# MegviiRobot/CamLaserCalibraTool

Hardware: AMD Instinct MI355X
Metric: residual+Jacobian evals/s (LM solve, 1e6-obs synthetic point-to-plane problem per GPU) (higher is better)
Workload: dtype f64

## Files before the change

camlasercalibratool_amd/csrc/clc_coop.hpp:

```cpp
#pragma once
#include "clc_lmuni.hpp"
#include "clc_resident.hpp"

namespace clc {

constexpr int COOP_WGS = 256, COOP_GROUPS = 8, COOP_PER_GROUP = COOP_WGS / COOP_GROUPS, COOP_ROW_WORDS = 64;
constexpr int COOP_SMALL_WGS = 32;
#ifndef CLC_COOP_A_STRIDE
#define CLC_COOP_A_STRIDE 64
#endif
#ifndef CLC_COOP_B_STRIDE
#define CLC_COOP_B_STRIDE 64
#endif
constexpr int COOP_A_STRIDE = CLC_COOP_A_STRIDE, COOP_B_STRIDE = CLC_COOP_B_STRIDE;
constexpr int COOP_NW = 4, COOP_NL = 64 * COOP_NW;
constexpr int COOP_THREADS = COOP_NL + 64;
constexpr int COOP_STATUS_ABORT = -1;
constexpr int COOP_PR = 16, COOP_PL = 24;
constexpr int COOP_PR_Z = 10, COOP_PL_Z = 16;
constexpr unsigned long long COOP_CENSUS_TICKS = 20000ull;
constexpr unsigned long long COOP_TIMEOUT_TICKS = 100000ull;
constexpr int COOP_DONE_OK = 1, COOP_DONE_ABORT = 2;
#ifndef CLC_COOP_POLL_SLEEP
#define CLC_COOP_POLL_SLEEP 1
#endif
#ifndef CLC_COOP_D1
#define CLC_COOP_D1 900
#endif
#ifndef CLC_COOP_D2
#define CLC_COOP_D2 2200
#endif

#ifndef CLC_COOP_GRP
#define CLC_COOP_GRP 8
#endif
#ifndef CLC_COOP_REPLICAS
#define CLC_COOP_REPLICAS 1
#endif
constexpr int COOP_REPLICAS = CLC_COOP_REPLICAS;
constexpr unsigned long long COOP_ABORT_CHECK_TICKS = 2000ull;
struct CoopBoard {
  unsigned long long a[2][COOP_WGS][COOP_A_STRIDE];
  unsigned long long b[2][COOP_REPLICAS][COOP_GROUPS][COOP_B_STRIDE];
  unsigned long long ctl[8];
};

typedef unsigned int v4u __attribute__((ext_vector_type(4)));
constexpr int COOP_SC1 = 16;
__device__ __forceinline__ __amdgpu_buffer_rsrc_t coop_rsrc(CoopBoard* board) {
  return __builtin_amdgcn_make_buffer_rsrc(board, 0, (int)sizeof(CoopBoard), 0x00020000);
}
__device__ __forceinline__ void coop_put(__amdgpu_buffer_rsrc_t rs, const unsigned int row_byte, const int e, const double v, const unsigned int tag) {
  v4u w;
  w[0] = tag; w[1] = (unsigned int)__double2hiint(v); w[2] = tag; w[3] = (unsigned int)__double2loint(v);
  __builtin_amdgcn_raw_buffer_store_b128(w, rs, row_byte + 16u * (unsigned int)e, 0, COOP_SC1);
}
__device__ __forceinline__ v4u coop_get(__amdgpu_buffer_rsrc_t rs, const unsigned int byte) {
  return __builtin_amdgcn_raw_buffer_load_b128(rs, byte, 0, COOP_SC1);
}
__device__ __forceinline__ bool coop_valid(const v4u w, const unsigned int tag) { return w[0] == tag && w[2] == tag; }
__device__ __forceinline__ double coop_value(const v4u w) { return __hiloint2double((int)w[1], (int)w[3]); }
__device__ __forceinline__ unsigned int coop_row_a(const int par, const int wg) {
  return (unsigned int)(offsetof(CoopBoard, a) + ((size_t)(par * COOP_WGS + wg) * COOP_A_STRIDE) * 8);
}
__device__ __forceinline__ unsigned int coop_row_b(const int par, const int copy, const int grp) {
  return (unsigned int)(offsetof(CoopBoard, b) + ((size_t)((par * COOP_REPLICAS + copy) * COOP_GROUPS + grp) * COOP_B_STRIDE) * 8);
}
__device__ __forceinline__ void coop_wait_until(const long long t) {
  while (clock64() < t) __builtin_amdgcn_s_sleep(2);
}

#ifdef CLC_STAMPS
constexpr int COOP_STAMP_PASSES = 16, COOP_STAMP_PER_PASS = 12, COOP_STAMP_SLOTS = COOP_STAMP_PER_PASS * COOP_STAMP_PASSES + 2;
static __device__ long long clc_coop_stamp_buf[4][2][COOP_STAMP_SLOTS];
#define COOP_STAMP(slot)                                                                                                     \
  do {                                                                                                                       \
    if (lane == 0 && (wave == 0 || wave >= COOP_NW - 1) && (wg == 0 || wg == 7 || wg == 8 || wg == 255) && (slot) < COOP_STAMP_SLOTS)  \
      clc_coop_stamp_buf[wg == 0 ? 0 : wg == 7 ? 1 : wg == 8 ? 2 : 3][wave == COOP_NW - 1 ? 1 : 0][slot] = clock64();          \
  } while (0)
#else
#define COOP_STAMP(slot) do {} while (0)
#endif

__device__ __forceinline__ void wave_reduce_to_rows(double (&acc)[NACC], double (&u)[7]) {
  double r[14];
#pragma unroll
  for (int i = 0; i < 14; ++i) {
    double x = acc[i], y = acc[i + 14];
    swap_halves(x, y);
    r[i] = x + y;
  }
#pragma unroll
  for (int i = 0; i < 7; ++i) {
    double x = r[i], y = r[i + 7];
    swap_rows(x, y);
    u[i] = x + y;
  }
}

template <bool WITH_LOSS, bool NT, bool WITH_Z = false, bool ONE_HOP = false>
__global__ __launch_bounds__(COOP_THREADS) void coop_solve_kernel(
    const double* __restrict__ xyl, const double* __restrict__ zl, const unsigned int* __restrict__ res_row, const ResLane* __restrict__ lane_desc,
    const double* __restrict__ groups, const int uni_ppl, const clc_options opt, const Pose7 pose0, clc_iteration* __restrict__ trace,
    const int trace_cap, CoopBoard* __restrict__ board, const unsigned int tag0, double* __restrict__ pose_out,
    clc_summary* __restrict__ summary_out, double* __restrict__ results, int32_t* __restrict__ host_done, const int n_wgs) {
  constexpr int NW = COOP_NW, NL = COOP_NL, PR = WITH_Z ? COOP_PR_Z : COOP_PR, PL = WITH_Z ? COOP_PL_Z : COOP_PL, NP = PR + PL;
  constexpr int CH = WITH_Z ? 4 : 6, NCH = (PL + CH - 1) / CH;
  static_assert(NW == 4, "the row tail maps the four 16-lane rows of a wave onto the four point waves");
  using Moments = typename std::conditional<WITH_Z, RowMoments3, RowMoments>::type;
  __shared__ v2d sh_pts[PL * NL];
  __shared__ double sh_ptz[WITH_Z ? PL * NL : 1];
  __shared__ double sh_state[LM_STATE_WORDS];
  __shared__ __attribute__((aligned(16))) double sh_tot[64];
  __shared__ double sh_red[NW * 7 * 64];
  __shared__ __attribute__((aligned(16))) double sh_pub[LM_PUB_WORDS];
  const int wg = blockIdx.x, tid = threadIdx.x, lane = tid & 63, wave = tid >> 6;
  const int cap = opt.max_num_iterations + 2;
#ifdef CLC_STAMPS
  int stamp_pass = 0;
  COOP_STAMP(COOP_STAMP_PER_PASS * COOP_STAMP_PASSES);
#endif

  if (wave == NW) {
    constexpr bool one_hop = ONE_HOP;
    constexpr int groups = ONE_HOP ? 1 : COOP_GROUPS;
    const int grp = ONE_HOP ? 0 : wg % COOP_GROUPS;
    const bool leader = ONE_HOP || wg < COOP_GROUPS;
    clc_iteration* const tr = wg == 0 ? trace : nullptr;
    const int tr_cap = wg == 0 ? trace_cap : 0;
    LmState& st = *reinterpret_cast<LmState*>(sh_state);
    const __amdgpu_buffer_rsrc_t rs = coop_rsrc(board);
    LmU S;
    {
      double x0[7];
#pragma unroll
      for (int i = 0; i < 7; ++i) x0[i] = pose0.v[i];
      lmu_init(S, st, opt, x0, lane);
      lmu_publish(sh_pub, x0, CLC_RUNNING, lane);
    }
    __syncthreads();
    bool aborted = false;

    const long long d1 = board->ctl[1] ? (long long)board->ctl[1] : (ONE_HOP ? 1900 : CLC_COOP_D1), d2 = board->ctl[2] ? (long long)board->ctl[2] : CLC_COOP_D2;
    for (int k = 0;; ++k) {
      __syncthreads();
      const unsigned int tag = tag0 + (unsigned int)k;
      const int par = k & 1;
      const int h = lane >> 5, e = (lane & 31) < NACC ? (lane & 31) : NACC - 1;
      const bool mine = lane < NACC;
      const unsigned long long limit = k == 0 ? COOP_CENSUS_TICKS : COOP_TIMEOUT_TICKS;
      bool fine = true;
      const long long t_a = clock64();
      if (ONE_HOP) {
        if (k > 0) lmu_pre(S, st, opt, sh_tot, tr, tr_cap, lane);
        COOP_STAMP(COOP_STAMP_PER_PASS * stamp_pass + 11);
      }
      if (leader) {
        coop_wait_until(t_a + d1);
        v4u w[16];
        const unsigned int base = coop_row_a(par, grp + groups * 16 * h) + 16u * (unsigned int)e;
        constexpr unsigned int row_step = (unsigned int)(groups * COOP_A_STRIDE * 8);
        const unsigned long long t0 = wall_clock64();
        for (;;) {
          bool ok = true;
          unsigned int bo = base;
          asm volatile("" : "+v"(bo));
#pragma unroll
          for (int i = 0; i < 16; ++i) w[i] = coop_get(rs, bo + (unsigned int)i * row_step);
#pragma unroll
          for (int i = 0; i < 16; ++i) ok = ok && coop_valid(w[i], tag);
          if (__all(ok)) break;
          const unsigned long long waited = wall_clock64() - t0;
          if (waited > COOP_ABORT_CHECK_TICKS) {
            unsigned int co = (unsigned int)offsetof(CoopBoard, ctl);
            asm volatile("" : "+v"(co));
            if (waited > limit || coop_get(rs, co)[0] == tag0) { fine = false; break; }
          }
          __builtin_amdgcn_s_sleep(CLC_COOP_POLL_SLEEP);
        }
        COOP_STAMP(COOP_STAMP_PER_PASS * stamp_pass + 3);
        double s = coop_value(w[0]);
#pragma unroll
        for (int i = 1; i < 16; ++i) s += coop_value(w[i]);
        double s_lo = s, s_hi = s;
        swap_halves(s_lo, s_hi);
        if (one_hop) {
          if (mine) sh_tot[32 * (1 - S.hx) + lane] = s_lo + s_hi;
        } else if (mine && fine) {
          int so = lane;
          asm volatile("" : "+v"(so));
#pragma unroll
          for (int r = 0; r < COOP_REPLICAS; ++r) coop_put(rs, coop_row_b(par, (r + grp) % COOP_REPLICAS, grp), so, s_lo + s_hi, tag);
        }
        COOP_STAMP(COOP_STAMP_PER_PASS * stamp_pass + 4);
      }
      if (!ONE_HOP) {
        if (k > 0 && !leader) lmu_pre(S, st, opt, sh_tot, tr, tr_cap, lane);
        if (!leader) COOP_STAMP(COOP_STAMP_PER_PASS * stamp_pass + 11);
      }
      if (fine && !one_hop) {
        coop_wait_until(t_a + d2);
        const unsigned int base = coop_row_b(par, wg % COOP_REPLICAS, 4 * h) + 16u * (unsigned int)e;
        const unsigned long long t0 = wall_clock64();
        bool pre_due = k > 0 && leader;
        v4u w[4];
        for (;;) {
          bool ok = true;
          unsigned int bo = base;
          asm volatile("" : "+v"(bo));
#pragma unroll
          for (int i = 0; i < 4; ++i) w[i] = coop_get(rs, bo + (unsigned int)(i * COOP_B_STRIDE * 8));
          if (pre_due) {
            asm volatile("" ::: "memory");
            __builtin_amdgcn_sched_barrier(0);
            lmu_pre(S, st, opt, sh_tot, tr, tr_cap, lane);
            __builtin_amdgcn_sched_barrier(0);
            COOP_STAMP(COOP_STAMP_PER_PASS * stamp_pass + 11);
            pre_due = false;
          }
#pragma unroll
          for (int i = 0; i < 4; ++i) ok = ok && coop_valid(w[i], tag);
          if (__all(ok)) break;
          const unsigned long long waited = wall_clock64() - t0;
          if (waited > COOP_ABORT_CHECK_TICKS) {
            unsigned int co = (unsigned int)offsetof(CoopBoard, ctl);
            asm volatile("" : "+v"(co));
            if (waited > limit || coop_get(rs, co)[0] == tag0) { fine = false; break; }
          }
          __builtin_amdgcn_s_sleep(CLC_COOP_POLL_SLEEP);
        }
        COOP_STAMP(COOP_STAMP_PER_PASS * stamp_pass + 5);
        double s = coop_value(w[0]);
#pragma unroll
        for (int i = 1; i < 4; ++i) s += coop_value(w[i]);
        double s_lo = s, s_hi = s;
        swap_halves(s_lo, s_hi);
        if (mine) sh_tot[32 * (1 - S.hx) + lane] = s_lo + s_hi;
      }
      __builtin_amdgcn_fence(__ATOMIC_RELEASE, "wavefront");
      __builtin_amdgcn_wave_barrier();
      __builtin_amdgcn_fence(__ATOMIC_ACQUIRE, "wavefront");
      COOP_STAMP(COOP_STAMP_PER_PASS * stamp_pass + 6);
      if (fine) {
        lmu_post(k == 0, S, opt, sh_tot, sh_pub, tr, tr_cap, lane);
        if (S.status == CLC_RUNNING && k >= cap) {
          S.status = CLC_FAILURE;
          lmu_publish_status(sh_pub, CLC_FAILURE, lane);
        }
      } else {
        if (lane == 0) __hip_atomic_store(reinterpret_cast<unsigned int*>(&board->ctl[0]), tag0, __ATOMIC_RELAXED, __HIP_MEMORY_SCOPE_AGENT);
        lmu_publish_status(sh_pub, COOP_STATUS_ABORT, lane);
        aborted = true;
      }
      COOP_STAMP(COOP_STAMP_PER_PASS * stamp_pass + 7);
      __syncthreads();
      if (aborted || S.status != CLC_RUNNING) break;
#ifdef CLC_STAMPS
      ++stamp_pass;
#endif
    }
    if (wg == 0) {
      if (!aborted) {
        lmu_finish(S, st, opt, sh_tot, tr, tr_cap, lane);
        if (lane == 0) batched_write_outcome(st, 0, pose_out, summary_out, results);
      }
      if (lane == 0) __hip_atomic_store(host_done, aborted ? COOP_DONE_ABORT : COOP_DONE_OK, __ATOMIC_RELEASE, __HIP_MEMORY_SCOPE_SYSTEM);
    }
    return;
  }

  __builtin_amdgcn_s_setprio(2);
  const __amdgpu_buffer_rsrc_t rs_p = coop_rsrc(board);
  unsigned int row0;
  int ppl;
  if (uni_ppl >= 0) {
    row0 = (unsigned int)wg * (unsigned int)uni_ppl;
    ppl = uni_ppl;
  } else {
    row0 = res_row[wg];
    ppl = __builtin_amdgcn_readfirstlane((int)(res_row[wg + 1] - row0));
  }
  const ResLane dl = lane_desc[(size_t)wg * NL + tid];
  const v2d* __restrict__ src = reinterpret_cast<const v2d*>(xyl) + (size_t)row0 * NL + tid;
  const int j_last = ppl > 0 ? ppl - 1 : 0;
  const double* __restrict__ srcz = WITH_Z ? zl + (size_t)row0 * NL + tid : nullptr;
  v2d lds_v[PL];
  double lds_z[WITH_Z ? PL : 1];
  const bool use_lds = (ppl + CLC_COOP_GRP - 1) / CLC_COOP_GRP * CLC_COOP_GRP > PR;
  if (use_lds) {
#pragma unroll
    for (int i = 0; i < PL; ++i) {
      const int j = PR + i;
      lds_v[i] = res_load<NT>(src + (size_t)(j < j_last ? j : j_last) * NL);
      if (WITH_Z) lds_z[i] = srcz[(size_t)(j < j_last ? j : j_last) * NL];
    }
  }
  v2d reg[PR];
  double regz[WITH_Z ? PR : 1];
#pragma unroll
  for (int j = 0; j < PR; ++j) {
    reg[j] = res_load<NT>(src + (size_t)(j < j_last ? j : j_last) * NL);
    if (WITH_Z) regz[j] = srcz[(size_t)(j < j_last ? j : j_last) * NL];
  }
  if (use_lds) {
#pragma unroll
    for (int i = 0; i < PL; ++i) {
      v2d v = lds_v[i];
      double vz = WITH_Z ? lds_z[i] : 0.0;
      if (PR + i >= ppl) { v[0] = 0.0; v[1] = 0.0; vz = 0.0; }
      sh_pts[i * NL + tid] = v;
      if (WITH_Z) sh_ptz[i * NL + tid] = vz;
    }
  }
  const double* __restrict__ gp = groups + (size_t)dl.gid * GROUP_DOUBLES;
  const int cnt = dl.cnt;
  double pl_nx = 0.0, pl_ny = 0.0, pl_nz = 0.0, pl_d = 0.0, pl_s2 = 0.0;
  if (cnt > 0) {
    const v2d a = *reinterpret_cast<const v2d*>(gp);
    const v2d b = *reinterpret_cast<const v2d*>(gp + 2);
    const double s = gp[4];
    pl_nx = a[0]; pl_ny = a[1]; pl_nz = b[0]; pl_d = b[1]; pl_s2 = s * s;
  }
  const double inv_lf2 = make_uniform(1.0 / (opt.loss_scale_factor * opt.loss_scale_factor));
  constexpr int GRP = CLC_COOP_GRP;
  const int ppl_up = (ppl + GRP - 1) / GRP * GRP;
  const int ppl_eff = ppl_up < NP ? ppl_up : NP;
#ifndef CLC_COOP_PAD_ANALYTIC
#define CLC_COOP_PAD_ANALYTIC 0
#endif
  constexpr bool PAD_ANALYTIC = CLC_COOP_PAD_ANALYTIC != 0;
  static_assert(!(PAD_ANALYTIC && WITH_Z), "the analytic padding correction is written for (x, y) slots only");
  const int cnt_m = cnt > 0 ? cnt : ppl_eff;
  int cmin = cnt_m;
#pragma unroll
  for (int off = 32; off >= 1; off >>= 1) {
    const int o2 = __shfl_xor(cmin, off, 64);
    cmin = o2 < cmin ? o2 : cmin;
  }
  cmin = __builtin_amdgcn_readfirstlane(cmin);
  __syncthreads();
  COOP_STAMP(COOP_STAMP_PER_PASS * COOP_STAMP_PASSES + 1);
#pragma unroll
  for (int j = 0; j < PR; ++j)
    if (j >= ppl) { reg[j][0] = 0.0; reg[j][1] = 0.0; if (WITH_Z) regz[j] = 0.0; }

  for (int k = 0;; ++k) {
    COOP_STAMP(COOP_STAMP_PER_PASS * stamp_pass);
    int t = tid;
    asm volatile("" : "+v"(t));
    RowPlane q;
    {
      const lds_cv2d* pb = lds_opaque(sh_pub);
      const v2d p0 = pb[0], p1 = pb[1], p2 = pb[2], p3 = pb[3], p4 = pb[4], p5 = pb[5], p6 = pb[6];
      int status = __double2loint(p6[0]);
      asm volatile("" : "+v"(status) : "v"(p0), "v"(p1), "v"(p2), "v"(p3), "v"(p4), "v"(p5));
      if (status != CLC_RUNNING) break;
      q.nx = pl_nx; q.ny = pl_ny; q.nz = pl_nz; q.s2 = pl_s2;
      q.mx = fma(p3[0], pl_nz, fma(p1[1], pl_ny, p0[0] * pl_nx));
      q.my = fma(p3[1], pl_nz, fma(p2[0], pl_ny, p0[1] * pl_nx));
      q.mz = fma(p4[0], pl_nz, fma(p2[1], pl_ny, p1[0] * pl_nx));
      q.c0 = fma(p5[1], pl_nz, fma(p5[0], pl_ny, fma(p4[1], pl_nx, pl_d)));
    }
    v2d buf[2][CH];
    double bufz[2][WITH_Z ? CH : 1];
    if (use_lds) {
#pragma unroll
      for (int u = 0; u < CH; ++u)
        if (u < PL) {
          buf[0][u] = sh_pts[u * NL + t];
          if (WITH_Z) bufz[0][u] = sh_ptz[u * NL + t];
        }
    }
#ifdef CLC_STAMPS
    asm volatile("" :: "v"(q.mx), "v"(q.c0));
    COOP_STAMP(COOP_STAMP_PER_PASS * stamp_pass + 8);
#endif
    Moments M;
    lane_moments_reset<WITH_LOSS>(M);
#pragma unroll
    for (int j0 = 0; j0 < NP; j0 += GRP) {
      if (j0 < ppl) {
        if (PAD_ANALYTIC || j0 + GRP <= cmin) {
#pragma unroll
          for (int j = j0; j < j0 + GRP && j < NP; ++j) {
            if (j >= PR && (j - PR) % CH == 0 && (j - PR) / CH + 1 < NCH) {
              const int c1 = (j - PR) / CH + 1;
#pragma unroll
              for (int u = 0; u < CH; ++u)
                if (c1 * CH + u < PL) {
                  buf[c1 & 1][u] = sh_pts[(c1 * CH + u) * NL + t];
                  if (WITH_Z) bufz[c1 & 1][u] = sh_ptz[(c1 * CH + u) * NL + t];
                }
            }
            const v2d v = j < PR ? reg[j < PR ? j : 0] : buf[((j - PR) / CH) & 1][(j - PR) % CH];
            const double vz = !WITH_Z ? 0.0 : (j < PR ? regz[j < PR ? j : 0] : bufz[((j - PR) / CH) & 1][(j - PR) % CH]);
            lane_point<WITH_LOSS>(q, inv_lf2, v[0], v[1], vz, M, j == j0 + GRP - 1);
          }
        } else {
#pragma unroll
          for (int j = j0; j < j0 + GRP && j < NP; ++j) {
            if (j >= PR && (j - PR) % CH == 0 && (j - PR) / CH + 1 < NCH) {
              const int c1 = (j - PR) / CH + 1;
#pragma unroll
              for (int u = 0; u < CH; ++u)
                if (c1 * CH + u < PL) {
                  buf[c1 & 1][u] = sh_pts[(c1 * CH + u) * NL + t];
                  if (WITH_Z) bufz[c1 & 1][u] = sh_ptz[(c1 * CH + u) * NL + t];
                }
            }
            const v2d v = j < PR ? reg[j < PR ? j : 0] : buf[((j - PR) / CH) & 1][(j - PR) % CH];
            const double vz = !WITH_Z ? 0.0 : (j < PR ? regz[j < PR ? j : 0] : bufz[((j - PR) / CH) & 1][(j - PR) % CH]);
            lane_point_masked<WITH_LOSS>(q, j < cnt_m, inv_lf2, v[0], v[1], vz, M, j == j0 + GRP - 1);
          }
        }
      }
    }
    double lp = 0.0;
    if (PAD_ANALYTIC) {
      const int npad = ppl_eff - cnt;
      const double np = (double)npad;
      const double c0 = q.c0;
      if (WITH_LOSS) {
        const double sum_p = fma(c0 * c0, inv_lf2, 1.0);
        const double w_p = rcp_ge1(sum_p);
        const double cs = npad > 0 ? np * w_p : 0.0;
        M.S0 -= cs;
        M.T0 = fma(-cs, c0, M.T0);
        int e;
        const double m = frexp_pos(sum_p, e);
        lp = npad > 0 ? np * log_mant_exp(m, e) : 0.0;
      } else {
        const double cs = npad > 0 ? np : 0.0;
        M.S0 -= cs;
        M.T0 = fma(-cs, c0, M.T0);
        M.prod = fma(-cs * c0, c0, M.prod);
      }
    } else {
      lane_pad_correction<WITH_LOSS>(M, (double)(ppl_eff - cnt_m));
    }
#ifdef CLC_STAMPS
    asm volatile("" :: "v"(M.S0), "v"(M.Tx), "v"(M.prod));
    COOP_STAMP(COOP_STAMP_PER_PASS * stamp_pass + 9);
#endif
    double acc[NACC];
#pragma unroll
    for (int i = 0; i < NACC; ++i) acc[i] = 0.0;
    lane_flush<WITH_LOSS>(q, M, acc);
    if (PAD_ANALYTIC && WITH_LOSS) acc[27] = fma(-q.s2, lp, acc[27]);
#ifdef CLC_STAMPS
    asm volatile("" :: "v"(acc[0]), "v"(acc[20]), "v"(acc[27]));
    COOP_STAMP(COOP_STAMP_PER_PASS * stamp_pass + 10);
#endif
    {
      double u[7];
      wave_reduce_to_rows(acc, u);
#pragma unroll
      for (int i = 0; i < 7; ++i) sh_red[(wave * 7 + i) * 64 + lane] = u[i];
    }
    COOP_STAMP(COOP_STAMP_PER_PASS * stamp_pass + 1);
    __syncthreads();
    {
      const unsigned int tag = tag0 + (unsigned int)k;
      const int s0 = ((lane >> 4) * 7) * 64 + 16 * wave + (lane & 15);
      double v[8];
#pragma unroll
      for (int i = 0; i < 7; ++i) v[i] = sh_red[s0 + i * 64];
      v[7] = 0.0;
      double r[4], s[2];
#pragma unroll
      for (int i = 0; i < 4; ++i) {
        double x = v[i], y = v[i + 4];
        swap_halves(x, y);
        r[i] = x + y;
      }
#pragma unroll
      for (int i = 0; i < 2; ++i) {
        double x = r[i], y = r[i + 2];
        swap_rows(x, y);
        s[i] = x + y;
      }
#pragma unroll
      for (int i = 0; i < 2; ++i) {
        double w = s[i];
        w += dpp_read<0xB1>(w);
        w += dpp_read<0x4E>(w);
        w += dpp_read<0x141>(w);
        w += dpp_read<0x140>(w);
        s[i] = w;
      }
      if ((lane & 15) == 0) {
        const int rho = lane >> 4;
        const unsigned int row = coop_row_a(k & 1, wg);
#pragma unroll
        for (int i = 0; i < 2; ++i) {
          const int e = i + 2 * (rho & 1) + 4 * (rho >> 1);
          if (e < 7) coop_put(rs_p, row, 7 * wave + e, s[i], tag);
        }
      }
    }
    COOP_STAMP(COOP_STAMP_PER_PASS * stamp_pass + 2);
    __syncthreads();
#ifdef CLC_STAMPS
    ++stamp_pass;
#endif
  }
}

}
```

Baseline: 154.4 billion.

## Move group-leader gather into a dedicated extra wave per workgroup

Adds a sixth wave to each workgroup that, on the first COOP_GROUPS workgroups, polls the stage-A board rows, sums the group partials and publishes them to the stage-B board. The control wave no longer does the leader gather itself, so every workgroup runs lmu_pre and the stage-B poll the same way and the leader's pre-step work no longer serialises with its gather. The D1/D2 spin delays are retuned to fit the new timing. In exchange each workgroup launches 64 more threads, which adds register and occupancy pressure and extra __syncthreads coordination between the waves.

Result: faster. 159.7 billion, median of 6 (+3.4%).

```diff
diff --git a/camlasercalibratool_amd/csrc/clc_coop.hpp b/camlasercalibratool_amd/csrc/clc_coop.hpp
--- a/camlasercalibratool_amd/csrc/clc_coop.hpp
+++ b/camlasercalibratool_amd/csrc/clc_coop.hpp
@@ -14,7 +14,7 @@
 #endif
 constexpr int COOP_A_STRIDE = CLC_COOP_A_STRIDE, COOP_B_STRIDE = CLC_COOP_B_STRIDE;
 constexpr int COOP_NW = 4, COOP_NL = 64 * COOP_NW;
-constexpr int COOP_THREADS = COOP_NL + 64;
+constexpr int COOP_THREADS = COOP_NL + 128;
 constexpr int COOP_STATUS_ABORT = -1;
 constexpr int COOP_PR = 16, COOP_PL = 24;
 constexpr int COOP_PR_Z = 10, COOP_PL_Z = 16;
@@ -25,10 +25,10 @@
 #define CLC_COOP_POLL_SLEEP 1
 #endif
 #ifndef CLC_COOP_D1
-#define CLC_COOP_D1 900
+#define CLC_COOP_D1 1200
 #endif
 #ifndef CLC_COOP_D2
-#define CLC_COOP_D2 2200
+#define CLC_COOP_D2 1400
 #endif
 
 #ifndef CLC_COOP_GRP
@@ -96,6 +96,44 @@
     swap_rows(x, y);
     u[i] = x + y;
   }
+}
+
+template <int NR>
+__device__ __forceinline__ bool coop_poll(const __amdgpu_buffer_rsrc_t rs, const unsigned int base, const unsigned int step, const unsigned int tag,
+                                          const unsigned int tag0, const unsigned long long limit, v4u (&w)[NR]) {
+  const unsigned long long t0 = wall_clock64();
+  for (;;) {
+    bool ok = true;
+    unsigned int bo = base;
+    asm volatile("" : "+v"(bo));
+#pragma unroll
+    for (int i = 0; i < NR; ++i) w[i] = coop_get(rs, bo + (unsigned int)i * step);
+#pragma unroll
+    for (int i = 0; i < NR; ++i) ok = ok && coop_valid(w[i], tag);
+    if (__all(ok)) return true;
+    const unsigned long long waited = wall_clock64() - t0;
+    if (waited > COOP_ABORT_CHECK_TICKS) {
+      unsigned int co = (unsigned int)offsetof(CoopBoard, ctl);
+      asm volatile("" : "+v"(co));
+      if (waited > limit || coop_get(rs, co)[0] == tag0) return false;
+    }
+    __builtin_amdgcn_s_sleep(CLC_COOP_POLL_SLEEP);
+  }
+}
+
+template <int GROUPS>
+__device__ __forceinline__ bool coop_gather_group(const __amdgpu_buffer_rsrc_t rs, const int par, const int grp, const int lane, const unsigned int tag,
+                                                  const unsigned int tag0, const unsigned long long limit, double& row) {
+  const int h = lane >> 5, e = (lane & 31) < NACC ? (lane & 31) : NACC - 1;
+  v4u w[16];
+  const bool fine = coop_poll<16>(rs, coop_row_a(par, grp + GROUPS * 16 * h) + 16u * (unsigned int)e, (unsigned int)(GROUPS * COOP_A_STRIDE * 8), tag, tag0, limit, w);
+  double s = coop_value(w[0]);
+#pragma unroll
+  for (int i = 1; i < 16; ++i) s += coop_value(w[i]);
+  double s_lo = s, s_hi = s;
+  swap_halves(s_lo, s_hi);
+  row = s_lo + s_hi;
+  return fine;
 }
 
 template <bool WITH_LOSS, bool NT, bool WITH_Z = false, bool ONE_HOP = false>
@@ -121,11 +159,39 @@
   COOP_STAMP(COOP_STAMP_PER_PASS * COOP_STAMP_PASSES);
 #endif
 
+  if (wave == NW + 1) {
+    if (ONE_HOP || wg >= COOP_GROUPS) return;
+    const __amdgpu_buffer_rsrc_t rs = coop_rsrc(board);
+    const long long d1 = board->ctl[1] ? (long long)board->ctl[1] : CLC_COOP_D1;
+    const int grp = wg;
+    __syncthreads();
+    for (int k = 0;; ++k) {
+      __syncthreads();
+      const long long t_a = clock64();
+      const unsigned int tag = tag0 + (unsigned int)k;
+      const int par = k & 1;
+      coop_wait_until(t_a + d1);
+      double row;
+      const bool fine = coop_gather_group<COOP_GROUPS>(rs, par, grp, lane, tag, tag0, k == 0 ? COOP_CENSUS_TICKS : COOP_TIMEOUT_TICKS, row);
+      COOP_STAMP(COOP_STAMP_PER_PASS * stamp_pass + 3);
+      if (fine) {
+        if (lane < NACC) {
+#pragma unroll
+          for (int r = 0; r < COOP_REPLICAS; ++r) coop_put(rs, coop_row_b(par, (r + grp) % COOP_REPLICAS, grp), lane, row, tag);
+        }
+      } else if (lane == 0) {
+        __hip_atomic_store(reinterpret_cast<unsigned int*>(&board->ctl[0]), tag0, __ATOMIC_RELAXED, __HIP_MEMORY_SCOPE_AGENT);
+      }
+      COOP_STAMP(COOP_STAMP_PER_PASS * stamp_pass + 4);
+      __syncthreads();
+      if (reinterpret_cast<const volatile int*>(sh_pub + 12)[0] != CLC_RUNNING) return;
+#ifdef CLC_STAMPS
+      ++stamp_pass;
+#endif
+    }
+  }
+
   if (wave == NW) {
-    constexpr bool one_hop = ONE_HOP;
-    constexpr int groups = ONE_HOP ? 1 : COOP_GROUPS;
-    const int grp = ONE_HOP ? 0 : wg % COOP_GROUPS;
-    const bool leader = ONE_HOP || wg < COOP_GROUPS;
     clc_iteration* const tr = wg == 0 ? trace : nullptr;
     const int tr_cap = wg == 0 ? trace_cap : 0;
     LmState& st = *reinterpret_cast<LmState*>(sh_state);
@@ -141,94 +207,28 @@
     __syncthreads();
     bool aborted = false;
 
-    const long long d1 = board->ctl[1] ? (long long)board->ctl[1] : (ONE_HOP ? 1900 : CLC_COOP_D1), d2 = board->ctl[2] ? (long long)board->ctl[2] : CLC_COOP_D2;
+    const long long d = ONE_HOP ? (board->ctl[1] ? (long long)board->ctl[1] : 1900) : (board->ctl[2] ? (long long)board->ctl[2] : CLC_COOP_D2);
     for (int k = 0;; ++k) {
       __syncthreads();
       const unsigned int tag = tag0 + (unsigned int)k;
       const int par = k & 1;
-      const int h = lane >> 5, e = (lane & 31) < NACC ? (lane & 31) : NACC - 1;
       const bool mine = lane < NACC;
       const unsigned long long limit = k == 0 ? COOP_CENSUS_TICKS : COOP_TIMEOUT_TICKS;
-      bool fine = true;
+      bool fine;
       const long long t_a = clock64();
+      if (k > 0) lmu_pre(S, st, opt, sh_tot, tr, tr_cap, lane);
+      COOP_STAMP(COOP_STAMP_PER_PASS * stamp_pass + 11);
+      coop_wait_until(t_a + d);
       if (ONE_HOP) {
-        if (k > 0) lmu_pre(S, st, opt, sh_tot, tr, tr_cap, lane);
-        COOP_STAMP(COOP_STAMP_PER_PASS * stamp_pass + 11);
-      }
-      if (leader) {
-        coop_wait_until(t_a + d1);
-        v4u w[16];
-        const unsigned int base = coop_row_a(par, grp + groups * 16 * h) + 16u * (unsigned int)e;
-        constexpr unsigned int row_step = (unsigned int)(groups * COOP_A_STRIDE * 8);
-        const unsigned long long t0 = wall_clock64();
-        for (;;) {
-          bool ok = true;
-          unsigned int bo = base;
-          asm volatile("" : "+v"(bo));
-#pragma unroll
-          for (int i = 0; i < 16; ++i) w[i] = coop_get(rs, bo + (unsigned int)i * row_step);
-#pragma unroll
-          for (int i = 0; i < 16; ++i) ok = ok && coop_valid(w[i], tag);
-          if (__all(ok)) break;
-          const unsigned long long waited = wall_clock64() - t0;
-          if (waited > COOP_ABORT_CHECK_TICKS) {
-            unsigned int co = (unsigned int)offsetof(CoopBoard, ctl);
-            asm volatile("" : "+v"(co));
-            if (waited > limit || coop_get(rs, co)[0] == tag0) { fine = false; break; }
-          }
-          __builtin_amdgcn_s_sleep(CLC_COOP_POLL_SLEEP);
-        }
+        double row;
+        fine = coop_gather_group<1>(rs, par, 0, lane, tag, tag0, limit, row);
         COOP_STAMP(COOP_STAMP_PER_PASS * stamp_pass + 3);
-        double s = coop_value(w[0]);
-#pragma unroll
-        for (int i = 1; i < 16; ++i) s += coop_value(w[i]);
-        double s_lo = s, s_hi = s;
-        swap_halves(s_lo, s_hi);
-        if (one_hop) {
-          if (mine) sh_tot[32 * (1 - S.hx) + lane] = s_lo + s_hi;
-        } else if (mine && fine) {
-          int so = lane;
-          asm volatile("" : "+v"(so));
-#pragma unroll
-          for (int r = 0; r < COOP_REPLICAS; ++r) coop_put(rs, coop_row_b(par, (r + grp) % COOP_REPLICAS, grp), so, s_lo + s_hi, tag);
-        }
+        if (mine) sh_tot[32 * (1 - S.hx) + lane] = row;
         COOP_STAMP(COOP_STAMP_PER_PASS * stamp_pass + 4);
-      }
-      if (!ONE_HOP) {
-        if (k > 0 && !leader) lmu_pre(S, st, opt, sh_tot, tr, tr_cap, lane);
-        if (!leader) COOP_STAMP(COOP_STAMP_PER_PASS * stamp_pass + 11);
-      }
-      if (fine && !one_hop) {
-        coop_wait_until(t_a + d2);
-        const unsigned int base = coop_row_b(par, wg % COOP_REPLICAS, 4 * h) + 16u * (unsigned int)e;
-        const unsigned long long t0 = wall_clock64();
-        bool pre_due = k > 0 && leader;
+      } else {
+        const int h = lane >> 5, e = (lane & 31) < NACC ? (lane & 31) : NACC - 1;
         v4u w[4];
-        for (;;) {
-          bool ok = true;
-          unsigned int bo = base;
-          asm volatile("" : "+v"(bo));
-#pragma unroll
-          for (int i = 0; i < 4; ++i) w[i] = coop_get(rs, bo + (unsigned int)(i * COOP_B_STRIDE * 8));
-          if (pre_due) {
-            asm volatile("" ::: "memory");
-            __builtin_amdgcn_sched_barrier(0);
-            lmu_pre(S, st, opt, sh_tot, tr, tr_cap, lane);
-            __builtin_amdgcn_sched_barrier(0);
-            COOP_STAMP(COOP_STAMP_PER_PASS * stamp_pass + 11);
-            pre_due = false;
-          }
-#pragma unroll
-          for (int i = 0; i < 4; ++i) ok = ok && coop_valid(w[i], tag);
-          if (__all(ok)) break;
-          const unsigned long long waited = wall_clock64() - t0;
-          if (waited > COOP_ABORT_CHECK_TICKS) {
-            unsigned int co = (unsigned int)offsetof(CoopBoard, ctl);
-            asm volatile("" : "+v"(co));
-            if (waited > limit || coop_get(rs, co)[0] == tag0) { fine = false; break; }
-          }
-          __builtin_amdgcn_s_sleep(CLC_COOP_POLL_SLEEP);
-        }
+        fine = coop_poll<4>(rs, coop_row_b(par, wg % COOP_REPLICAS, 4 * h) + 16u * (unsigned int)e, (unsigned int)(COOP_B_STRIDE * 8), tag, tag0, limit, w);
         COOP_STAMP(COOP_STAMP_PER_PASS * stamp_pass + 5);
         double s = coop_value(w[0]);
 #pragma unroll
```
